# Napoliee/Expressive-FastSpeech2-Mandarin

Measured on AMD Instinct MI355X. Metric: mel-frames/sec/GPU (batch-64 synth) at 1/2/4/8 MI355X; RTF, higher is better.
Workload: dtype bf16; 1 GPU; cfg2: batch=64 x 64 phonemes per GPU, ESD-Chinese-Singing-MFA model.yaml, FastSpeech2.forward eval bf16; global_batch=64, seq_len=64, mel_frames_per_gpu_batch=24883, T_max=430, parallelism=dp1 (independent shards, no collective), hip_graph=True

## Files before the change

### expressive-fastspeech2-mandarin_amd/csrc/enc_block.hip

```cpp
#include "cond.h"
#include "fs2_common.h"

namespace {

typedef __amdgpu_buffer_rsrc_t rsrc_t;
typedef short s16x4 __attribute__((ext_vector_type(4)));

constexpr int D = 256, NQKV = 768, LMAX = 64, DK = 128, NT = 512;
constexpr int kUnit = 4096;

__device__ __forceinline__ rsrc_t rsrc(const void *p, uint32_t bytes) {
  return __builtin_amdgcn_make_buffer_rsrc(const_cast<void *>(p), (short)0, (int)bytes, 0x00020000);
}
__device__ __forceinline__ int kv_swz(int row) { return ((row & 7) << 1) | ((row >> 3) & 1); }
__device__ __forceinline__ int kv_off(int row, int chunk) { return row * 256 + ((chunk ^ kv_swz(row)) << 4); }
__device__ __forceinline__ float max_nn(float a, float b) { return __builtin_fmaxf(a, b); }
__device__ __forceinline__ float rows_sum(float v) {
  auto a = __builtin_amdgcn_permlane16_swap(__float_as_uint(v), __float_as_uint(v), false, false);
  const float s1 = __uint_as_float(a[0]) + __uint_as_float(a[1]);
  auto b = __builtin_amdgcn_permlane32_swap(__float_as_uint(s1), __float_as_uint(s1), false, false);
  return __uint_as_float(b[0]) + __uint_as_float(b[1]);
}
__device__ __forceinline__ float rows_max(float v) {
  auto a = __builtin_amdgcn_permlane16_swap(__float_as_uint(v), __float_as_uint(v), false, false);
  const float s1 = max_nn(__uint_as_float(a[0]), __uint_as_float(a[1]));
  auto b = __builtin_amdgcn_permlane32_swap(__float_as_uint(s1), __float_as_uint(s1), false, false);
  return max_nn(__uint_as_float(b[0]), __uint_as_float(b[1]));
}

__device__ __forceinline__ void bar() {
  __builtin_amdgcn_s_waitcnt(0xC07F);
  __builtin_amdgcn_sched_barrier(0);
  __builtin_amdgcn_s_barrier();
  __builtin_amdgcn_sched_barrier(0);
}

struct EncBlockArgs {
  const bf16 *x;
  const int64_t *lens;
  int B, L;
  const bf16 *wqkv;
  const float *bqkv;
  const bf16 *wfc;
  const float *bfc, *gamma, *beta;
  float eps, scale_log2;
  bf16 *out;
  const int64_t *tokens;
  const float *emb, *pe;
  int vocab, T_mel;
  int32_t *bad;
  uint8_t *src_mask;
  const int64_t *mel_lens;
  uint8_t *mel_mask;
  int *cnt;
  char *part;
  uint32_t part_bytes;
  CondArgs cond;
  int ncond, ncx;
};

constexpr int XP = D * 2 + 16;
constexpr int QP = DK * 2 + 16;
constexpr int X_OFF = 0;
constexpr int Q_OFF = X_OFF + LMAX * XP;
constexpr int K_OFF = Q_OFF + 2 * LMAX * QP;
constexpr int V_OFF = K_OFF + 2 * LMAX * 256;
constexpr int RED_OFF = V_OFF + 2 * LMAX * 256;
constexpr int VEC_OFF = RED_OFF + 2 * LMAX * 8 * 4;
constexpr int SMEM = VEC_OFF + (NQKV + 3 * D) * 4;
static_assert(2 * LMAX * QP >= LMAX * XP, "o fits the Q region");
static_assert(SMEM <= 163840, "LDS");

#ifndef ENC_TRACE
#define ENC_TRACE 0
#endif

__device__ __attribute__((noinline)) void cond_role(const CondArgs &a, int bx, int by, int tid, float *sm) {
  cond_tile(a, bx, by, tid, sm);
}

template <bool EMBED, bool COND = false>
__global__ __launch_bounds__(NT, 1) void enc_attn_block_kernel(EncBlockArgs p) {
  __shared__ __attribute__((aligned(16))) char smem[SMEM];
  uint64_t tst[10];
  int ntst = 0;
  auto stamp = [&]() {
    if (ENC_TRACE) {
      __builtin_amdgcn_sched_barrier(0);
      tst[ntst++] = __builtin_readcyclecounter();
      __builtin_amdgcn_sched_barrier(0);
    }
  };
// ... 590 lines not shown
#pragma unroll
      for (int mb = 0; mb < 4; ++mb)
        other[i][mb] = __builtin_bit_cast(f32x4, __builtin_amdgcn_raw_buffer_load_b128(pr, pofs(hh ^ 1, i, mb), 0, 16));
#pragma unroll
    for (int i = 0; i < 2; ++i)
#pragma unroll
      for (int mb = 0; mb < 4; ++mb) fa[i][mb] = hh == 0 ? fa[i][mb] + other[i][mb] : other[i][mb] + fa[i][mb];
  }
  float *red = reinterpret_cast<float *>(smem + RED_OFF);
  float part[4];
#pragma unroll
  for (int mb = 0; mb < 4; ++mb) {
    const int m = 16 * mb + li;
    float sm = 0.f;
#pragma unroll
    for (int i = 0; i < 2; ++i) {
      const int n = 16 * (2 * w + i) + 4 * g;
      const float4 bb = *reinterpret_cast<const float4 *>(vfc + n);
      const bf16x4 xv = *reinterpret_cast<const bf16x4 *>(smem + X_OFF + m * XP + n * 2);
      f32x4 v = fa[i][mb];
      v[0] = v[0] + bb.x + (float)xv[0];
      v[1] = v[1] + bb.y + (float)xv[1];
      v[2] = v[2] + bb.z + (float)xv[2];
      v[3] = v[3] + bb.w + (float)xv[3];
      fa[i][mb] = v;
      sm += (v[0] + v[1]) + (v[2] + v[3]);
    }
    part[mb] = rows_sum(sm);
  }
  auto reduce = [&](float (&pv)[4], float (&tot)[4], int pass) {
    float *rb = red + pass * LMAX * 8;
    if (g == 0) {
#pragma unroll
      for (int mb = 0; mb < 4; ++mb) rb[(16 * mb + li) * 8 + w] = pv[mb];
    }
    bar();
#pragma unroll
    for (int mb = 0; mb < 4; ++mb) {
      const float4 a = *reinterpret_cast<const float4 *>(rb + (16 * mb + li) * 8);
      const float4 c = *reinterpret_cast<const float4 *>(rb + (16 * mb + li) * 8 + 4);
      tot[mb] = ((a.x + a.y) + (a.z + a.w)) + ((c.x + c.y) + (c.z + c.w));
    }
  };
  float mean[4], var[4];
  reduce(part, mean, 0);
#pragma unroll
  for (int mb = 0; mb < 4; ++mb) {
    mean[mb] *= 1.0f / D;
    float sm = 0.f;
#pragma unroll
    for (int i = 0; i < 2; ++i) {
      f32x4 d = fa[i][mb];
#pragma unroll
      for (int j = 0; j < 4; ++j) d[j] -= mean[mb];
      fa[i][mb] = d;
      sm += (d[0] * d[0] + d[1] * d[1]) + (d[2] * d[2] + d[3] * d[3]);
    }
    part[mb] = rows_sum(sm);
  }
  reduce(part, var, 1);
#pragma unroll
  for (int mb = 0; mb < 4; ++mb) {
    const int m = 16 * mb + li;
    const float rstd = 1.0f / sqrtf(var[mb] * (1.0f / D) + p.eps);
    const float keep = m < len ? 1.0f : 0.0f;
#pragma unroll
    for (int i = 0; i < 2; ++i) {
      const int n = 16 * (2 * w + i) + 4 * g;
      const float4 gg = *reinterpret_cast<const float4 *>(vg + n);
      const float4 be = *reinterpret_cast<const float4 *>(vb + n);
      const f32x4 d = fa[i][mb];
      const bf16x4 o = {(bf16)((d[0] * rstd * gg.x + be.x) * keep), (bf16)((d[1] * rstd * gg.y + be.y) * keep),
                        (bf16)((d[2] * rstd * gg.z + be.z) * keep), (bf16)((d[3] * rstd * gg.w + be.w) * keep)};
      *reinterpret_cast<bf16x4 *>(smem + X_OFF + m * XP + n * 2) = o;
    }
  }
  __builtin_amdgcn_s_waitcnt(0xC07F);
  bar();
  uint4 *orow = reinterpret_cast<uint4 *>(p.out + (size_t)xrow0 * D);
  for (int i = tid; i < L * (D * 2 / 16); i += NT) {
    const int m = i >> 5, c = i & 31;
    orow[i] = *reinterpret_cast<const uint4 *>(smem + X_OFF + m * XP + c * 16);
  }
}

}

static int enc_block_launch(const void *x, const int64_t *tokens, const float *emb, int vocab, const float *pe,
                            int32_t *bad_ids, const int64_t *lens, int B, int L, const void *wqkv, const float *bqkv,
                            const void *wfc, const float *bfc, const float *gamma, const float *beta, float eps, int H,
                            int dk, float temperature, void *out, uint8_t *src_mask, const int64_t *mel_lens, int T_mel,
                            uint8_t *mel_mask, const fs2_cond_desc *cond, void *ws, int64_t ws_bytes,
                            fs2_stream_t stream) {
  const bool embed = tokens != nullptr;
  if ((!embed && x == nullptr) || (embed && (emb == nullptr || pe == nullptr || vocab <= 0)) || lens == nullptr ||
      wqkv == nullptr || bqkv == nullptr || wfc == nullptr || bfc == nullptr || gamma == nullptr || beta == nullptr ||
      out == nullptr || !(temperature > 0.f))
    return FS2_EINVAL;
  if (B < 0 || L < 0 || (mel_mask != nullptr && (mel_lens == nullptr || T_mel < 0))) return FS2_EINVAL;
  if (H != 2 || dk != DK || L > LMAX) return FS2_EUNSUPPORTED;
  if (x == out) return FS2_EINVAL;
  if (B == 0 || L == 0) return FS2_OK;
  if ((int64_t)B * L * D * 2 >= (1LL << 31)) return FS2_EUNSUPPORTED;
  EncBlockArgs a{};
  a.x = reinterpret_cast<const bf16 *>(x);
  a.lens = lens;
  a.B = B;
  a.L = L;
  a.wqkv = reinterpret_cast<const bf16 *>(wqkv);
  a.bqkv = bqkv;
  a.wfc = reinterpret_cast<const bf16 *>(wfc);
  a.bfc = bfc;
  a.gamma = gamma;
  a.beta = beta;
  a.eps = eps;
  a.scale_log2 = 1.4426950408889634f / temperature;
  a.out = reinterpret_cast<bf16 *>(out);
  a.tokens = tokens;
  a.emb = emb;
  a.pe = pe;
  a.vocab = vocab;
  a.bad = bad_ids;
  a.src_mask = src_mask;
  a.mel_lens = mel_lens;
  a.T_mel = T_mel;
  a.mel_mask = mel_mask;
  a.cnt = reinterpret_cast<int *>(ws);
  a.part = ws != nullptr ? static_cast<char *>(ws) + 4096 : nullptr;
  a.part_bytes = (uint32_t)(ws_bytes > 4096 ? ws_bytes - 4096 : 0);
  a.ncond = a.ncx = 0;
  if (cond != nullptr && (cond->speaker_table != nullptr || cond->emo_table != nullptr)) {
    if (!embed) return FS2_EINVAL;
    if (cond->speaker_table != nullptr && (cond->speakers == nullptr || cond->spk_out == nullptr || cond->n_speaker <= 0))
      return FS2_EINVAL;
    if (cond->emo_table != nullptr &&
        (cond->emotions == nullptr || cond->arousals == nullptr || cond->valences == nullptr || cond->aro_table == nullptr ||
         cond->val_table == nullptr || cond->lin_w == nullptr || cond->lin_b == nullptr || cond->emo_out == nullptr ||
         cond->n_emo <= 0 || cond->n_aro <= 0 || cond->n_val <= 0))
      return FS2_EINVAL;
    const int dc = cond->emo_table != nullptr ? cond->d_emo + cond->d_aro + cond->d_val : 0;
    if ((int64_t)kCondU * (dc + 256) * 4 > SMEM) return FS2_EUNSUPPORTED;
    a.cond = CondArgs{cond->speakers, cond->speaker_table, cond->n_speaker, cond->emotions, cond->emo_table, cond->n_emo,
                      cond->d_emo, cond->arousals, cond->aro_table, cond->n_aro, cond->d_aro, cond->valences,
                      cond->val_table, cond->n_val, cond->d_val, cond->lin_w, cond->lin_b, B, D, cond->spk_out,
                      cond->emo_out};
    a.ncx = D / 64;
    a.ncond = a.ncx * ((B + kCondU - 1) / kCondU);
  }
  const bool half = !ENC_TRACE && a.ncond == 0 && ws != nullptr && B <= 1024 &&
                    (int64_t)B * 2 * 65536 + 4096 <= ws_bytes;
  const unsigned nhalf = (unsigned)(((B + 7) / 8) * 16);
  if (half && embed)
    hipLaunchKernelGGL(enc_attn_half_kernel<true>, dim3(nhalf), dim3(NT), 0, as_stream(stream), a);
  else if (half)
    hipLaunchKernelGGL(enc_attn_half_kernel<false>, dim3(nhalf), dim3(NT), 0, as_stream(stream), a);
  else if (embed && a.ncond > 0)
    hipLaunchKernelGGL((enc_attn_block_kernel<true, true>), dim3((unsigned)(B + a.ncond)), dim3(NT), 0,
                       as_stream(stream), a);
  else if (embed)
    hipLaunchKernelGGL(enc_attn_block_kernel<true>, dim3((unsigned)B), dim3(NT), 0, as_stream(stream), a);
  else
    hipLaunchKernelGGL(enc_attn_block_kernel<false>, dim3((unsigned)B), dim3(NT), 0, as_stream(stream), a);
  FS2_CHECK_LAUNCH();
  return FS2_OK;
}

extern "C" int fs2_enc_attn_block(const void *x, const int64_t *lens, int B, int L, const void *wqkv, const float *bqkv,
                                  const void *wfc, const float *bfc, const float *gamma, const float *beta, float eps,
                                  int H, int dk, float temperature, void *out, void *ws, int64_t ws_bytes,
                                  fs2_stream_t stream) {
  return enc_block_launch(x, nullptr, nullptr, 0, nullptr, nullptr, lens, B, L, wqkv, bqkv, wfc, bfc, gamma, beta, eps, H,
                          dk, temperature, out, nullptr, nullptr, 0, nullptr, nullptr, ws, ws_bytes, stream);
}

extern "C" int fs2_enc_embed_attn_block(const int64_t *tokens, const float *emb, int vocab, const float *pe,
                                        int32_t *bad_ids, const int64_t *lens, int B, int L, const void *wqkv,
                                        const float *bqkv, const void *wfc, const float *bfc, const float *gamma,
                                        const float *beta, float eps, int H, int dk, float temperature, void *out,
                                        uint8_t *src_mask, const int64_t *mel_lens, int T_mel, uint8_t *mel_mask,
                                        const fs2_cond_desc *cond, void *ws, int64_t ws_bytes, fs2_stream_t stream) {
  if (tokens == nullptr) return FS2_EINVAL;
  return enc_block_launch(nullptr, tokens, emb, vocab, pe, bad_ids, lens, B, L, wqkv, bqkv, wfc, bfc, gamma, beta, eps,
                          H, dk, temperature, out, src_mask, mel_lens, T_mel, mel_mask, cond, ws, ws_bytes, stream);
}
```

### expressive-fastspeech2-mandarin_amd/csrc/ffn_wide.hip

```cpp
#include <cstdlib>
#include <type_traits>
#include <utility>

#include "conv_common.h"
#include "fs2_common.h"

#ifndef WIDE_TRACE
#define WIDE_TRACE 0
#endif

namespace {

constexpr int kWD = 256;
constexpr int kWUnit = 4096;
constexpr int kWLgkm0 = 0xC07F;

template <int N, typename Fn, int... I>
__device__ __forceinline__ void wfor_impl(Fn &&f, std::integer_sequence<int, I...>) {
  (f(std::integral_constant<int, I>{}), ...);
}
template <int N, typename Fn>
__device__ __forceinline__ void wfor(Fn &&f) {
  wfor_impl<N>(f, std::make_integer_sequence<int, N>{});
}
// ... 165 lines not shown
#pragma unroll
    for (int mb = 0; mb < MB; ++mb) acc[jb][mb] = f32x4{0.f, 0.f, 0.f, 0.f};
  auto issue = [&](auto CI, auto TI, bf16x8 (&f)[MB]) {
    constexpr int c = decltype(CI)::value, t = decltype(TI)::value, off = (c % NSLOT) * CH;
#pragma unroll
    for (int mb = 0; mb < MB; ++mb) {
      uint32_t a;
      asm volatile("v_bfe_u32 %0, %1, %2, 16" : "=v"(a) : "v"(adp[t][mb >> 1]), "n"((mb & 1) * 16));
      f[mb] = *reinterpret_cast<const bf16x8 *>(smem + a + off);
    }
  };
  auto mma = [&](const bf16x8 (&fa)[2], const bf16x8 (&fb)[MB]) {
#pragma unroll
    for (int mb = 0; mb < MB; ++mb)
#pragma unroll
      for (int jb = 0; jb < 2; ++jb)
        acc[jb][mb] = __builtin_amdgcn_mfma_f32_16x16x32_bf16(fa[jb], fb[mb], acc[jb][mb], 0, 0, 0);
  };
  bf16x8 f0[MB], f1[MB];
  issue(std::integral_constant<int, 0>{}, std::integral_constant<int, 0>{}, f0);
  wfor<NCH>([&](auto CI) {
    constexpr int c = decltype(CI)::value;
    wfor<KS>([&](auto TI) {
      constexpr int t = decltype(TI)::value;
      constexpr int kk = c * KS + t;
      if constexpr (t + 1 < KS) {
        if constexpr (kk & 1)
          issue(CI, std::integral_constant<int, t + 1>{}, f0);
        else
          issue(CI, std::integral_constant<int, t + 1>{}, f1);
      } else if constexpr (c + 1 < NCH) {
        wait_chunk(std::integral_constant<int, c + 1>{});
        if constexpr (c + 2 < NCH) dma_chunk(std::integral_constant<int, c + 2>{});
        if constexpr (kk & 1)
          issue(std::integral_constant<int, c + 1>{}, std::integral_constant<int, 0>{}, f0);
        else
          issue(std::integral_constant<int, c + 1>{}, std::integral_constant<int, 0>{}, f1);
      }
      if constexpr (kk & 1)
        mma(pa[kk % RD], f1);
      else
        mma(pa[kk % RD], f0);
      if constexpr (kk + RD < NK) load_at(std::integral_constant<int, kk + RD>{});
    });
  });
  __builtin_amdgcn_s_waitcnt(kWLgkm0);
  __builtin_amdgcn_s_barrier();
  st.at();

  constexpr int HP = 144;
  const int hrow0 = rh * 128 + r16;
#pragma unroll
  for (int jb = 0; jb < 2; ++jb) {
    const float4 bb = jb == 0 ? bb0 : bb1;
#pragma unroll
    for (int mb = 0; mb < MB; ++mb) {
      const f32x4 v = acc[jb][mb];
      bf16x4 o;
      o[0] = (bf16)fmaxf(v[0] + bb.x, 0.f);
      o[1] = (bf16)fmaxf(v[1] + bb.y, 0.f);
      o[2] = (bf16)fmaxf(v[2] + bb.z, 0.f);
      o[3] = (bf16)fmaxf(v[3] + bb.w, 0.f);
      *reinterpret_cast<bf16x4 *>(smem + (hrow0 + 16 * mb) * HP + (hh * 32 + jb * 16 + 4 * hi) * 2) = o;
    }
  }
  __builtin_amdgcn_s_waitcnt(kWLgkm0);
  __syncthreads();
  const uint32_t hrow = (uint32_t)p.F * 2u;
  char *hb = reinterpret_cast<char *>(p.h);
#pragma unroll
  for (int i = 0; i < BM * 8 / 256; ++i) {
    const int e = tid + 256 * i, r = e >> 3, c = e & 7;
    if (m0 + r < M)
      *reinterpret_cast<uint4 *>(hb + (uint32_t)(m0 + r) * hrow + (uint32_t)(slice * 128 + c * 16)) =
          *reinterpret_cast<const uint4 *>(smem + r * HP + c * 16);
  }
  if (WIDE_TRACE) {
    asm volatile("s_waitcnt vmcnt(0)" ::: "memory");
    st.at();
    st.put(p.trace, L);
  }
}

template <int F>
__global__ __launch_bounds__(256, 1) void ffn_out_kernel(WideArgs p) {
  constexpr int NK = F / 32;
  constexpr int KW = NK / 4;
  constexpr int RED = 4 * 16 * 64 * 16;
  constexpr int VEC = RED;
  constexpr int OP = kWD * 2 + 16;
  static_assert(64 * OP <= RED, "staging fits");
  __shared__ __attribute__((aligned(16))) char smem[RED + 2048 + 16];
  Stamps st;
  st.at();

  const int tid = threadIdx.x, lane = tid & 63;
  const int w = __builtin_amdgcn_readfirstlane(tid >> 6);
  const int L = (blockIdx.x & 7) * (gridDim.x >> 3) + (blockIdx.x >> 3);
  const int tile = L >> 2, q = L & 3;
  if (tile >= p.ntiles) return;
  const int M = p.rows_dev != nullptr ? min(*p.rows_dev, p.M) : p.M;
  const int m0 = tile * 64;
  if (m0 >= M) return;
  const int T = p.T;
  const int hi = lane >> 4, r16 = lane & 15;
  if (w < 2)
    __builtin_amdgcn_raw_ptr_buffer_load_lds(make_rsrc(w == 0 ? p.gamma : p.beta, 1024),
                                             (__attribute__((address_space(3))) void *)(smem + VEC + w * 1024), 16,
                                             (uint32_t)lane * 16u, 0, 0, 0);

  const rsrc_t wr = make_rsrc(p.w, p.w_bytes);
  const rsrc_t hr = make_rsrc(p.h, p.h_bytes);
  bf16x8 wa[KW][4], hb[KW][4];
  const uint32_t wb = p.w_bytes - (uint32_t)(kWD * F * 2) + (uint32_t)((q * NK + w * KW) * kWUnit) + (uint32_t)lane * 16u;
  const uint32_t hrow = (uint32_t)F * 2u;
#pragma unroll
  for (int k = 0; k < KW; ++k) {
#pragma unroll
    for (int jb = 0; jb < 4; ++jb)
      wa[k][jb] = __builtin_bit_cast(bf16x8, __builtin_amdgcn_raw_buffer_load_b128(wr, wb + k * kWUnit + jb * 1024, 0, 0));
#pragma unroll
    for (int mb = 0; mb < 4; ++mb) {
      const int m = m0 + mb * 16 + r16;
      hb[k][mb] = __builtin_bit_cast(
          bf16x8, __builtin_amdgcn_raw_buffer_load_b128(
                      hr, m < M ? (uint32_t)m * hrow + (uint32_t)((w * KW + k) * 64 + hi * 16) : kOOB, 0, 0));
    }
  }
  const int m = m0 + 16 * w + r16;
  const bool mok = m < M;
  const rsrc_t xr = make_rsrc(p.x, p.x_bytes);
  const rsrc_t zr = make_rsrc(p.z, p.z_bytes);
  float4 b2v[4];
  uint2 xv[4];
#pragma unroll
  for (int jb = 0; jb < 4; ++jb) {
    const int n = 64 * q + 16 * jb + 4 * hi;
    b2v[jb] = *reinterpret_cast<const float4 *>(p.b2 + n);
    xv[jb] = bload8(xr, mok ? (uint32_t)m * (uint32_t)p.xs * 2u + (uint32_t)n * 2u : kOOB);
  }
  __builtin_amdgcn_sched_barrier(0);
  if (WIDE_TRACE) {
    asm volatile("s_waitcnt vmcnt(0)" ::: "memory");
    st.at();
  }
  f32x4 acc[4][4];
#pragma unroll
  for (int jb = 0; jb < 4; ++jb)
#pragma unroll
    for (int mb = 0; mb < 4; ++mb) acc[jb][mb] = f32x4{0.f, 0.f, 0.f, 0.f};
#pragma unroll
  for (int k = 0; k < KW; ++k)
#pragma unroll
    for (int mb = 0; mb < 4; ++mb)
#pragma unroll
      for (int jb = 0; jb < 4; ++jb)
        acc[jb][mb] = __builtin_amdgcn_mfma_f32_16x16x32_bf16(wa[k][jb], hb[k][mb], acc[jb][mb], 0, 0, 0);
  f32x4 *red = reinterpret_cast<f32x4 *>(smem);
#pragma unroll
  for (int jb = 0; jb < 4; ++jb)
#pragma unroll
    for (int mb = 0; mb < 4; ++mb) red[(w * 16 + jb * 4 + mb) * 64 + lane] = acc[jb][mb];
  __builtin_amdgcn_s_waitcnt(kWLgkm0);
  __builtin_amdgcn_s_barrier();
  st.at();
  f32x4 zv[4];
#pragma unroll
  for (int jb = 0; jb < 4; ++jb) {
    f32x4 s = red[(0 * 16 + jb * 4 + w) * 64 + lane];
#pragma unroll
    for (int ww = 1; ww < 4; ++ww) s += red[(ww * 16 + jb * 4 + w) * 64 + lane];
    zv[jb] = s;
  }
#pragma unroll
  for (int jb = 0; jb < 4; ++jb) {
    const int n = 64 * q + 16 * jb + 4 * hi;
    const bf16x4 x4 = __builtin_bit_cast(bf16x4, xv[jb]);
    f32x4 v = zv[jb];
    v[0] = v[0] + b2v[jb].x + (float)x4[0];
    v[1] = v[1] + b2v[jb].y + (float)x4[1];
    v[2] = v[2] + b2v[jb].z + (float)x4[2];
    v[3] = v[3] + b2v[jb].w + (float)x4[3];
    __builtin_amdgcn_raw_buffer_store_b128(__builtin_bit_cast(__attribute__((ext_vector_type(4))) unsigned, v), zr,
                                           mok ? ((uint32_t)m * kWD + (uint32_t)n) * 4u : kOOB, 0, 16);
  }
  asm volatile("s_waitcnt vmcnt(0)" ::: "memory");
  __syncthreads();
  st.at();
  int *flag = reinterpret_cast<int *>(smem + RED + 2048);
  if (tid == 0) {
    const int old = __hip_atomic_fetch_add(p.cnt + tile, 1, __ATOMIC_RELAXED, __HIP_MEMORY_SCOPE_AGENT);
    const int last = old == 3;
    if (last) __hip_atomic_store(p.cnt + tile, 0, __ATOMIC_RELAXED, __HIP_MEMORY_SCOPE_AGENT);
    *flag = last;
  }
  __syncthreads();
  st.at();
  if (!*flag) {
    st.put(p.trace, L);
    return;
  }

  if (mok) {
    f32x4 v[16];
#pragma unroll
    for (int i = 0; i < 16; ++i)
      v[i] = __builtin_bit_cast(f32x4, __builtin_amdgcn_raw_buffer_load_b128(
                                           zr, ((uint32_t)m * kWD + (uint32_t)(16 * i + 4 * hi)) * 4u, 0, 16));
    bool masked = false;
    int bb = 0;
    if (p.row_pos == nullptr) {
      bb = m / T;
      masked = p.lens != nullptr && (int64_t)(m - bb * T) >= p.lens[bb];
    }
    float4 a1[16], a2[16];
#pragma unroll
    for (int i = 0; i < 16; ++i) {
      const int n = 16 * i + 4 * hi;
      a1[i] = p.av1 != nullptr ? *reinterpret_cast<const float4 *>(p.av1 + (int64_t)bb * kWD + n) : make_float4(0.f, 0.f, 0.f, 0.f);
    }
    float s = 0.f;
#pragma unroll
    for (int i = 0; i < 16; ++i) s += (v[i][0] + v[i][1]) + (v[i][2] + v[i][3]);
    s += __shfl_xor(s, 16, 64);
    s += __shfl_xor(s, 32, 64);
    const float mean = s * (1.0f / 256.0f);
    float ss = 0.f;
#pragma unroll
    for (int i = 0; i < 16; ++i) {
      v[i] -= mean;
      ss += (v[i][0] * v[i][0] + v[i][1] * v[i][1]) + (v[i][2] * v[i][2] + v[i][3] * v[i][3]);
    }
    ss += __shfl_xor(ss, 16, 64);
    ss += __shfl_xor(ss, 32, 64);
    const float rstd = 1.0f / sqrtf(ss * (1.0f / 256.0f) + p.eps);
#pragma unroll
    for (int i = 0; i < 16; ++i) {
      const int n = 16 * i + 4 * hi;
      a2[i] = p.av2 != nullptr ? *reinterpret_cast<const float4 *>(p.av2 + (int64_t)bb * kWD + n) : make_float4(0.f, 0.f, 0.f, 0.f);
    }
    const float *vg = reinterpret_cast<const float *>(smem + VEC), *vb = vg + kWD;
#pragma unroll
    for (int i = 0; i < 16; ++i) {
      const int n = 16 * i + 4 * hi;
      const float4 g = *reinterpret_cast<const float4 *>(vg + n);
      const float4 be = *reinterpret_cast<const float4 *>(vb + n);
      float y[4] = {v[i][0] * rstd * g.x + be.x, v[i][1] * rstd * g.y + be.y, v[i][2] * rstd * g.z + be.z,
                    v[i][3] * rstd * g.w + be.w};
      if (masked) y[0] = y[1] = y[2] = y[3] = 0.f;
      if (p.av1 != nullptr) {
        y[0] += a1[i].x; y[1] += a1[i].y; y[2] += a1[i].z; y[3] += a1[i].w;
      }
      if (p.av2 != nullptr) {
        y[0] += a2[i].x; y[1] += a2[i].y; y[2] += a2[i].z; y[3] += a2[i].w;
      }
      const bf16x4 o = {(bf16)y[0], (bf16)y[1], (bf16)y[2], (bf16)y[3]};
      *reinterpret_cast<bf16x4 *>(smem + (16 * w + r16) * OP + n * 2) = o;
    }
  }
  __builtin_amdgcn_s_waitcnt(kWLgkm0);
  __builtin_amdgcn_s_barrier();
#pragma unroll
  for (int i = 0; i < 8; ++i) {
    const int e = tid + 256 * i, r = e >> 5, c = e & 31;
    if (m0 + r < M)
      *reinterpret_cast<uint4 *>(p.out + (int64_t)(m0 + r) * p.os + c * 8) =
          *reinterpret_cast<const uint4 *>(smem + r * OP + c * 16);
  }
  if (WIDE_TRACE) {
    asm volatile("s_waitcnt vmcnt(0)" ::: "memory");
    st.at();
    st.put(p.trace, L);
  }
}

}

extern "C" int fs2_ffn_wide(const fs2_ffn_desc *d, void *hidden, int64_t hidden_bytes, fs2_stream_t stream) {
  if (d == nullptr || d->x == nullptr || d->w == nullptr || d->b1 == nullptr || d->b2 == nullptr ||
      d->ln_gamma == nullptr || d->ln_beta == nullptr || d->out == nullptr || hidden == nullptr)
    return FS2_EINVAL;
  if (d->B < 0 || d->T < 0 || d->x_row_stride < kWD || (d->x_row_stride & 7) || d->out_row_stride < kWD ||
      (d->out_row_stride & 7))
    return FS2_EINVAL;
  if (d->D != kWD || !(d->F == 1024 || d->F == 512) || !(d->KS == 9 || d->KS == 3) || d->pad < 0 ||
      d->pad > d->KS - 1)
    return FS2_EUNSUPPORTED;
  if (d->wqkv != nullptr || d->pre_att != nullptr) return FS2_EUNSUPPORTED;
  if ((d->rows_dev == nullptr) != (d->row_pos == nullptr)) return FS2_EINVAL;
  if (d->rows_dev != nullptr && (d->lens != nullptr || d->addvec1 != nullptr || d->addvec2 != nullptr))
    return FS2_EINVAL;
  if (d->x == d->out || hidden == d->x || hidden == d->out) return FS2_EINVAL;
  const int64_t M64 = (int64_t)d->B * d->T;
  if (M64 > 0x7fffff00LL || d->rows_max < 0) return FS2_EINVAL;
  if (M64 == 0) return FS2_OK;
  const int64_t Mg = (d->rows_dev != nullptr && d->rows_max > 0 && d->rows_max < M64) ? d->rows_max : M64;
  const int64_t xb = M64 * d->x_row_stride * 2;
  const int64_t wb = ((int64_t)d->F * d->KS * kWD + (int64_t)kWD * d->F) * 2;
  const int64_t hb = Mg * d->F * 2;
  const int ntiles64 = (int)((Mg + 63) / 64);
  const int64_t zb = Mg * kWD * 4;
  if (xb >= (1LL << 31) || hb >= (1LL << 31) || hidden_bytes < hb) return FS2_EUNSUPPORTED;
  if (d->splitk_ws == nullptr || ntiles64 > 1024 || d->splitk_ws_bytes < 4096 + zb || zb >= (1LL << 31))
    return FS2_EINVAL;
  WideArgs p{};
  p.x = reinterpret_cast<const bf16 *>(d->x);
  p.xs = d->x_row_stride;
  p.x_bytes = (uint32_t)xb;
  p.w = reinterpret_cast<const bf16 *>(d->w);
  p.w_bytes = (uint32_t)wb;
  p.b1 = d->b1;
  p.b2 = d->b2;
  p.gamma = d->ln_gamma;
  p.beta = d->ln_beta;
  p.eps = d->ln_eps;
  p.lens = d->lens;
  p.av1 = d->addvec1;
  p.av2 = d->addvec2;
  p.rows_dev = d->rows_dev;
  p.row_pos = reinterpret_cast<const int2 *>(d->row_pos);
  p.M = (int)Mg;
  p.T = d->T;
  p.pad = d->pad;
  p.F = d->F;
  p.h = static_cast<bf16 *>(hidden);
  p.h_bytes = (uint32_t)hb;
  p.cnt = static_cast<int *>(d->splitk_ws);
  p.z = reinterpret_cast<float *>(static_cast<char *>(d->splitk_ws) + 4096);
  p.z_bytes = (uint32_t)zb;
  p.out = static_cast<bf16 *>(d->out);
  p.os = d->out_row_stride;
  if (WIDE_TRACE)
    p.trace = reinterpret_cast<uint64_t *>(static_cast<char *>(d->splitk_ws) + d->splitk_ws_bytes - 65536);
  hipStream_t s = as_stream(stream);
  p.nslices = d->F / 64;
  p.ntiles = (int)((Mg + 255) / 256);
  const int n1 = (p.nslices * p.ntiles + 7) & ~7;
  constexpr int kCUs = 256;
  const size_t solo = 32 * 1024;
  if (d->KS == 9)
    hipLaunchKernelGGL((ffn_hidden_kernel<9>), dim3(n1), dim3(256), n1 <= kCUs ? solo : 0, s, p);
  else
    hipLaunchKernelGGL((ffn_hidden_kernel<3>), dim3(n1), dim3(256), n1 <= kCUs ? solo : 0, s, p);
  FS2_CHECK_LAUNCH();
  p.ntiles = ntiles64;
  if (WIDE_TRACE) p.trace += 4096;
  const int n2 = (ntiles64 * 4 + 7) & ~7;
  if (d->F == 1024)
    hipLaunchKernelGGL((ffn_out_kernel<1024>), dim3(n2), dim3(256), 0, s, p);
  else
    hipLaunchKernelGGL((ffn_out_kernel<512>), dim3(n2), dim3(256), 0, s, p);
  FS2_CHECK_LAUNCH();
  return FS2_OK;
}
```

Before: 17.87 million mel-frames/s.

## Add row-split encoder attention and row-tiled FFN output kernels for small batches

Adds an encoder attention-block kernel that splits each sequence into four 16-row query blocks, so one batch launches about four times as many workgroups. Each block recomputes the full K/V projection but only its own Q rows, then does attention, output projection and LayerNorm. Also adds an FFN output kernel that tiles by 16 or 32 rows with the K reduction split across waves through LDS, instead of a split-K global workspace, and factors the LayerNorm epilogue into a shared helper. Both target small M where the existing kernels underfill the 256 CUs, at the cost of redundant K/V projection work and extra LDS reductions. Both are chosen by default and can be turned off with environment variables.

```diff
diff --git a/expressive-fastspeech2-mandarin_amd/csrc/enc_block.hip b/expressive-fastspeech2-mandarin_amd/csrc/enc_block.hip
--- a/expressive-fastspeech2-mandarin_amd/csrc/enc_block.hip
+++ b/expressive-fastspeech2-mandarin_amd/csrc/enc_block.hip
@@ -1,3 +1,5 @@
+#include <cstdlib>
+
 #include "cond.h"
 #include "fs2_common.h"
 
@@ -8,6 +10,7 @@
 
 constexpr int D = 256, NQKV = 768, LMAX = 64, DK = 128, NT = 512;
 constexpr int kUnit = 4096;
+constexpr int kRowsMaxB = 64;
 
 __device__ __forceinline__ rsrc_t rsrc(const void *p, uint32_t bytes) {
   return __builtin_amdgcn_make_buffer_rsrc(const_cast<void *>(p), (short)0, (int)bytes, 0x00020000);
@@ -764,6 +767,322 @@
     const int m = i >> 5, c = i & 31;
     orow[i] = *reinterpret_cast<const uint4 *>(smem + X_OFF + m * XP + c * 16);
   }
+}
+
+template <bool EMBED>
+__global__ __launch_bounds__(NT, 1) void enc_attn_rows_kernel(EncBlockArgs p) {
+  __shared__ __attribute__((aligned(16))) char smem[SMEM];
+  const int tid = threadIdx.x, lane = tid & 63;
+  const int w = __builtin_amdgcn_readfirstlane(tid >> 6);
+  const int g = lane >> 4, li = lane & 15;
+  const int bid = (blockIdx.x & 7) * (gridDim.x >> 3) + (blockIdx.x >> 3);
+  const int b = bid >> 2, q = bid & 3, L = p.L;
+  if (b >= p.B || 16 * q >= L) return;
+  const int64_t len64 = p.lens[b];
+  const int len = (int)(len64 < 0 ? 0 : (len64 > L ? L : len64));
+  const uint32_t xrow0 = (uint32_t)b * (uint32_t)L;
+  const int nrow = min(16, L - 16 * q);
+  uint4 *orow = reinterpret_cast<uint4 *>(p.out + ((size_t)xrow0 + 16 * q) * D);
+
+  if constexpr (EMBED) {
+    if (q == 0) {
+      if (p.src_mask != nullptr)
+        for (int t = tid; t < L; t += NT) p.src_mask[(int64_t)b * L + t] = (int64_t)t >= len64 ? 1 : 0;
+      if (p.mel_mask != nullptr) {
+        const int64_t ml = p.mel_lens[b];
+        for (int t = tid; t < p.T_mel; t += NT) p.mel_mask[(int64_t)b * p.T_mel + t] = (int64_t)t >= ml ? 1 : 0;
+      }
+    }
+  }
+  if (16 * q >= len) {
+    if constexpr (EMBED) {
+      if (q == 0 && p.bad != nullptr && tid < L) {
+        const int64_t tok = p.tokens[xrow0 + tid];
+        if (tok < 0 || tok >= p.vocab) atomicAdd(p.bad, 1);
+      }
+    }
+    if (tid < nrow * 32) orow[tid] = make_uint4(0u, 0u, 0u, 0u);
+    return;
+  }
+
+  if constexpr (!EMBED) {
+    const rsrc_t xr = rsrc(p.x, (uint32_t)p.B * (uint32_t)L * D * 2u);
+    for (int pc = w; pc < LMAX * XP / 1024; pc += 8) {
+      const int o = pc * 1024 + lane * 16, r = o / XP, within = o - r * XP;
+      const bool ok = r < L && within < D * 2;
+      __builtin_amdgcn_raw_ptr_buffer_load_lds(xr, (__attribute__((address_space(3))) void *)(smem + X_OFF + pc * 1024),
+                                               16, ok ? (xrow0 + r) * (uint32_t)(D * 2) + (uint32_t)within : 0x80000000u,
+                                               0, 0, 0);
+    }
+  }
+  if (w < 6) {
+    const float *src = w < 3 ? p.bqkv + 256 * w : w == 3 ? p.bfc : w == 4 ? p.gamma : p.beta;
+    __builtin_amdgcn_raw_ptr_buffer_load_lds(rsrc(src, 1024), (__attribute__((address_space(3))) void *)(smem + VEC_OFF + w * 1024),
+                                             16, (uint32_t)lane * 16u, 0, 0, 0);
+  }
+  const float *vqkv = reinterpret_cast<const float *>(smem + VEC_OFF);
+  const float *vfc = vqkv + NQKV, *vg = vfc + D, *vb = vg + D;
+
+  constexpr int NKV = 4, NQ = 2, NB1 = NKV + NQ, RING = 4;
+  const rsrc_t wq = rsrc(p.wqkv, (uint32_t)NQKV * D * 2u);
+  bf16x8 ring[RING][NB1];
+  auto gblock = [&](int i) { return i < NKV ? 16 + NKV * w + i : NQ * w + (i - NKV); };
+  auto wload = [&](int ks, bf16x8 (&dst)[NB1]) {
+    __builtin_amdgcn_sched_barrier(0);
+#pragma unroll
+    for (int i = 0; i < NB1; ++i) {
+      const int nb = gblock(i);
+      auto v = __builtin_amdgcn_raw_buffer_load_b128(
+          wq, (uint32_t)lane * 16u + (uint32_t)(nb & 3) * 1024u, (uint32_t)(((nb >> 2) * (D / 32) + ks) * kUnit), 0);
+      dst[i] = __builtin_bit_cast(bf16x8, v);
+    }
+    __builtin_amdgcn_sched_barrier(0);
+  };
+#pragma unroll
+  for (int ks = 0; ks < RING; ++ks) wload(ks, ring[ks]);
+  if constexpr (EMBED) {
+    for (int i = tid; i < LMAX * (D / 8); i += NT) {
+      const int r = i >> 5, c = (i & 31) * 8;
+      bf16x8 o;
+      if (r < L) {
+        const int64_t tok = p.tokens[xrow0 + r];
+        if (tok < 0 || tok >= p.vocab) {
+#pragma unroll
+          for (int k = 0; k < 8; ++k) o[k] = (bf16)__builtin_nanf("");
+          if (p.bad != nullptr && c == 0 && q == 0) atomicAdd(p.bad, 1);
+        } else {
+          float v[8], e[8];
+          load8(p.emb + tok * D + c, v);
+          load8(p.pe + (int64_t)r * D + c, e);
+#pragma unroll
+          for (int k = 0; k < 8; ++k) o[k] = (bf16)(v[k] + e[k]);
+        }
+      } else {
+#pragma unroll
+        for (int k = 0; k < 8; ++k) o[k] = (bf16)0.f;
+      }
+      *reinterpret_cast<bf16x8 *>(smem + X_OFF + r * XP + c * 2) = o;
+    }
+  }
+  asm volatile("s_waitcnt vmcnt(%0)" ::"n"((RING - 1) * NB1) : "memory");
+  __builtin_amdgcn_s_waitcnt(0xC07F);
+  bar();
+
+  f32x4 acc[NKV][4], qacc[NQ];
+#pragma unroll
+  for (int i = 0; i < NKV; ++i)
+#pragma unroll
+    for (int mb = 0; mb < 4; ++mb) acc[i][mb] = f32x4{0.f, 0.f, 0.f, 0.f};
+#pragma unroll
+  for (int i = 0; i < NQ; ++i) qacc[i] = f32x4{0.f, 0.f, 0.f, 0.f};
+  const int mq = 16 * q + li;
+#pragma unroll
+  for (int ks = 0; ks < D / 32; ++ks) {
+    bf16x8 xf[4];
+#pragma unroll
+    for (int mb = 0; mb < 4; ++mb)
+      xf[mb] = *reinterpret_cast<const bf16x8 *>(smem + X_OFF + (16 * mb + li) * XP + ks * 64 + g * 16);
+    const bf16x8 xq = *reinterpret_cast<const bf16x8 *>(smem + X_OFF + mq * XP + ks * 64 + g * 16);
+#pragma unroll
+    for (int i = 0; i < NKV; ++i)
+#pragma unroll
+      for (int mb = 0; mb < 4; ++mb)
+        acc[i][mb] = __builtin_amdgcn_mfma_f32_16x16x32_bf16(ring[ks % RING][i], xf[mb], acc[i][mb], 0, 0, 0);
+#pragma unroll
+    for (int i = 0; i < NQ; ++i)
+      qacc[i] = __builtin_amdgcn_mfma_f32_16x16x32_bf16(ring[ks % RING][NKV + i], xq, qacc[i], 0, 0, 0);
+    if (ks + RING < D / 32) wload(ks + RING, ring[ks % RING]);
+  }
+#pragma unroll
+  for (int i = 0; i < NKV; ++i) {
+    const int n = 16 * gblock(i) + 4 * g;
+    const float4 bb = *reinterpret_cast<const float4 *>(vqkv + n);
+    const int part = n >> 8, hh = (n >> 7) & 1, dim = n & 127;
+#pragma unroll
+    for (int mb = 0; mb < 4; ++mb) {
+      const int m = 16 * mb + li;
+      const f32x4 v = acc[i][mb];
+      const bf16x4 o = {(bf16)(v[0] + bb.x), (bf16)(v[1] + bb.y), (bf16)(v[2] + bb.z), (bf16)(v[3] + bb.w)};
+      *reinterpret_cast<bf16x4 *>(smem + (part == 1 ? K_OFF : V_OFF) + hh * LMAX * 256 + kv_off(m, dim >> 3) + (dim & 7) * 2) = o;
+    }
+  }
+#pragma unroll
+  for (int i = 0; i < NQ; ++i) {
+    const int n = 16 * gblock(NKV + i) + 4 * g;
+    const float4 bb = *reinterpret_cast<const float4 *>(vqkv + n);
+    const int hh = (n >> 7) & 1, dim = n & 127;
+    const f32x4 v = qacc[i];
+    const bf16x4 o = {(bf16)(v[0] + bb.x), (bf16)(v[1] + bb.y), (bf16)(v[2] + bb.z), (bf16)(v[3] + bb.w)};
+    *reinterpret_cast<bf16x4 *>(smem + Q_OFF + (hh * LMAX + mq) * QP + dim * 2) = o;
+  }
+  __builtin_amdgcn_s_waitcnt(0xC07F);
+  bar();
+
+  const rsrc_t wf = rsrc(p.wfc, (uint32_t)D * D * 2u);
+  bf16x8 fw[D / 32][2];
+#pragma unroll
+  for (int ks = 0; ks < D / 32; ++ks)
+#pragma unroll
+    for (int i = 0; i < 2; ++i) {
+      const int nb = 2 * w + i;
+      fw[ks][i] = __builtin_bit_cast(bf16x8, __builtin_amdgcn_raw_buffer_load_b128(
+                                                 wf, (uint32_t)lane * 16u + (uint32_t)(nb & 3) * 1024u,
+                                                 (uint32_t)(((nb >> 2) * (D / 32) + ks) * kUnit), 0));
+    }
+  f32x4 oacc[DK / 16];
+  float l_run = 0.f;
+  if (w < 2) {
+    const int h = w;
+    bf16x8 qf[4];
+#pragma unroll
+    for (int s = 0; s < 4; ++s)
+      qf[s] = *reinterpret_cast<const bf16x8 *>(smem + Q_OFF + (h * LMAX + mq) * QP + (32 * s + 8 * g) * 2);
+#pragma unroll
+    for (int i = 0; i < DK / 16; ++i) oacc[i] = f32x4{0.f, 0.f, 0.f, 0.f};
+    const char *Kb = smem + K_OFF + h * LMAX * 256;
+    const char *Vb = smem + V_OFF + h * LMAX * 256;
+    constexpr int NBK = LMAX / 16;
+    f32x4 sacc[NBK];
+#pragma unroll
+    for (int ni = 0; ni < NBK; ++ni) {
+      sacc[ni] = f32x4{0.f, 0.f, 0.f, 0.f};
+#pragma unroll
+      for (int s = 0; s < 4; ++s) {
+        const bf16x8 kf = *reinterpret_cast<const bf16x8 *>(Kb + kv_off(ni * 16 + li, 4 * s + g));
+        sacc[ni] = __builtin_amdgcn_mfma_f32_16x16x32_bf16(kf, qf[s], sacc[ni], 0, 0, 0);
+      }
+    }
+    const int lim = len - 4 * g;
+#pragma unroll
+    for (int ni = 0; ni < NBK; ++ni)
+#pragma unroll
+      for (int j = 0; j < 4; ++j)
+        if (ni * 16 + j >= lim) sacc[ni][j] = -INFINITY;
+    float mx = -INFINITY;
+#pragma unroll
+    for (int ni = 0; ni < NBK; ++ni) {
+      mx = max_nn(max_nn(mx, sacc[ni][0]), sacc[ni][1]);
+      mx = max_nn(max_nn(mx, sacc[ni][2]), sacc[ni][3]);
+    }
+    const float m_new = rows_max(mx);
+    const float mc = -m_new * p.scale_log2;
+    float sx = 0.f, sy = 0.f;
+    bf16x8 pf[NBK / 2];
+#pragma unroll
+    for (int ni = 0; ni < NBK; ++ni)
+#pragma unroll
+      for (int jp = 0; jp < 2; ++jp) {
+        const float px = __builtin_amdgcn_exp2f(__builtin_fmaf(sacc[ni][2 * jp], p.scale_log2, mc));
+        const float py = __builtin_amdgcn_exp2f(__builtin_fmaf(sacc[ni][2 * jp + 1], p.scale_log2, mc));
+        sx += px;
+        sy += py;
+        pf[ni >> 1][(ni & 1) * 4 + 2 * jp] = (bf16)px;
+        pf[ni >> 1][(ni & 1) * 4 + 2 * jp + 1] = (bf16)py;
+      }
+    l_run = rows_sum(sx + sy);
+    const int tq = li >> 2, tp = li & 3;
+#pragma unroll
+    for (int s2 = 0; s2 < NBK / 2; ++s2) {
+#pragma unroll
+      for (int h4 = 0; h4 < DK / 64; ++h4) {
+        bf16x8 vf[4];
+#pragma unroll
+        for (int i = 0; i < 4; ++i) {
+          const int nd = 4 * h4 + i;
+          const char *vp = Vb + kv_off(4 * g + tq, nd * 2 + (tp >> 1)) + (tp & 1) * 8 + s2 * 32 * 256;
+          auto lo = __builtin_amdgcn_ds_read_tr16_b64_v4i16((__attribute__((address_space(3))) s16x4 *)vp);
+          auto hi = __builtin_amdgcn_ds_read_tr16_b64_v4i16((__attribute__((address_space(3))) s16x4 *)(vp + 16 * 256));
+          __builtin_memcpy(&vf[i], &lo, 8);
+          __builtin_memcpy(reinterpret_cast<char *>(&vf[i]) + 8, &hi, 8);
+        }
+#pragma unroll
+        for (int i = 0; i < 4; ++i)
+          oacc[4 * h4 + i] = __builtin_amdgcn_mfma_f32_16x16x32_bf16(vf[i], pf[s2], oacc[4 * h4 + i], 0, 0, 0);
+      }
+    }
+  }
+  __builtin_amdgcn_s_waitcnt(0xC07F);
+  bar();
+  if (w < 2) {
+    const float inv = l_run > 0.f ? 1.0f / l_run : 0.f;
+#pragma unroll
+    for (int nd = 0; nd < DK / 16; ++nd) {
+      const bf16x4 o = {(bf16)(oacc[nd][0] * inv), (bf16)(oacc[nd][1] * inv), (bf16)(oacc[nd][2] * inv),
+                        (bf16)(oacc[nd][3] * inv)};
+      *reinterpret_cast<bf16x4 *>(smem + Q_OFF + mq * XP + (w * DK + nd * 16 + 4 * g) * 2) = o;
+    }
+  }
+  __builtin_amdgcn_s_waitcnt(0xC07F);
+  bar();
+
+  f32x4 fa[2];
+#pragma unroll
+  for (int i = 0; i < 2; ++i) fa[i] = f32x4{0.f, 0.f, 0.f, 0.f};
+#pragma unroll
+  for (int ks = 0; ks < D / 32; ++ks) {
+    const bf16x8 of = *reinterpret_cast<const bf16x8 *>(smem + Q_OFF + mq * XP + ks * 64 + g * 16);
+#pragma unroll
+    for (int i = 0; i < 2; ++i) fa[i] = __builtin_amdgcn_mfma_f32_16x16x32_bf16(fw[ks][i], of, fa[i], 0, 0, 0);
+  }
+  float *red = reinterpret_cast<float *>(smem + RED_OFF);
+  float part;
+  {
+    float s = 0.f;
+#pragma unroll
+    for (int i = 0; i < 2; ++i) {
+      const int n = 16 * (2 * w + i) + 4 * g;
+      const float4 bb = *reinterpret_cast<const float4 *>(vfc + n);
+      const bf16x4 xv = *reinterpret_cast<const bf16x4 *>(smem + X_OFF + mq * XP + n * 2);
+      f32x4 v = fa[i];
+      v[0] = v[0] + bb.x + (float)xv[0];
+      v[1] = v[1] + bb.y + (float)xv[1];
+      v[2] = v[2] + bb.z + (float)xv[2];
+      v[3] = v[3] + bb.w + (float)xv[3];
+      fa[i] = v;
+      s += (v[0] + v[1]) + (v[2] + v[3]);
+    }
+    part = rows_sum(s);
+  }
+  auto reduce = [&](float pv, int pass) {
+    float *rb = red + pass * LMAX * 8;
+    if (g == 0) rb[mq * 8 + w] = pv;
+    bar();
+    const float4 a = *reinterpret_cast<const float4 *>(rb + mq * 8);
+    const float4 c = *reinterpret_cast<const float4 *>(rb + mq * 8 + 4);
+    return ((a.x + a.y) + (a.z + a.w)) + ((c.x + c.y) + (c.z + c.w));
+  };
+  float mean = reduce(part, 0);
+  {
+    mean *= 1.0f / D;
+    float s = 0.f;
+#pragma unroll
+    for (int i = 0; i < 2; ++i) {
+      f32x4 d = fa[i];
+#pragma unroll
+      for (int j = 0; j < 4; ++j) d[j] -= mean;
+      fa[i] = d;
+      s += (d[0] * d[0] + d[1] * d[1]) + (d[2] * d[2] + d[3] * d[3]);
+    }
+    part = rows_sum(s);
+  }
+  const float var = reduce(part, 1);
+  {
+    const float rstd = 1.0f / sqrtf(var * (1.0f / D) + p.eps);
+    const float keep = mq < len ? 1.0f : 0.0f;
+#pragma unroll
+    for (int i = 0; i < 2; ++i) {
+      const int n = 16 * (2 * w + i) + 4 * g;
+      const float4 gg = *reinterpret_cast<const float4 *>(vg + n);
+      const float4 be = *reinterpret_cast<const float4 *>(vb + n);
+      const f32x4 d = fa[i];
+      const bf16x4 o = {(bf16)((d[0] * rstd * gg.x + be.x) * keep), (bf16)((d[1] * rstd * gg.y + be.y) * keep),
+                        (bf16)((d[2] * rstd * gg.z + be.z) * keep), (bf16)((d[3] * rstd * gg.w + be.w) * keep)};
+      *reinterpret_cast<bf16x4 *>(smem + X_OFF + mq * XP + n * 2) = o;
+    }
+  }
+  __builtin_amdgcn_s_waitcnt(0xC07F);
+  bar();
+  if (tid < nrow * 32) orow[tid] = *reinterpret_cast<const uint4 *>(smem + X_OFF + (16 * q + (tid >> 5)) * XP + (tid & 31) * 16);
 }
 
 }
@@ -832,7 +1151,14 @@
   const bool half = !ENC_TRACE && a.ncond == 0 && ws != nullptr && B <= 1024 &&
                     (int64_t)B * 2 * 65536 + 4096 <= ws_bytes;
   const unsigned nhalf = (unsigned)(((B + 7) / 8) * 16);
-  if (half && embed)
+  const char *erows = getenv("FS2_ENC_ROWS");
+  const bool rows = !ENC_TRACE && a.ncond == 0 && ws == nullptr && B <= kRowsMaxB && !(erows != nullptr && erows[0] == '0');
+  const unsigned nrows = (unsigned)((4 * B + 31) & ~31);
+  if (rows && embed)
+    hipLaunchKernelGGL(enc_attn_rows_kernel<true>, dim3(nrows), dim3(NT), 0, as_stream(stream), a);
+  else if (rows)
+    hipLaunchKernelGGL(enc_attn_rows_kernel<false>, dim3(nrows), dim3(NT), 0, as_stream(stream), a);
+  else if (half && embed)
     hipLaunchKernelGGL(enc_attn_half_kernel<true>, dim3(nhalf), dim3(NT), 0, as_stream(stream), a);
   else if (half)
     hipLaunchKernelGGL(enc_attn_half_kernel<false>, dim3(nhalf), dim3(NT), 0, as_stream(stream), a);
diff --git a/expressive-fastspeech2-mandarin_amd/csrc/ffn_wide.hip b/expressive-fastspeech2-mandarin_amd/csrc/ffn_wide.hip
--- a/expressive-fastspeech2-mandarin_amd/csrc/ffn_wide.hip
+++ b/expressive-fastspeech2-mandarin_amd/csrc/ffn_wide.hip
@@ -271,6 +271,200 @@
   }
 }
 
+__device__ __forceinline__ void ln_row(const WideArgs &p, f32x4 (&v)[16], int m, int hi, const char *vec, char *dst) {
+  bool masked = false;
+  int bb = 0;
+  if (p.row_pos == nullptr) {
+    bb = m / p.T;
+    masked = p.lens != nullptr && (int64_t)(m - bb * p.T) >= p.lens[bb];
+  }
+  float4 a1[16], a2[16];
+#pragma unroll
+  for (int i = 0; i < 16; ++i) {
+    const int n = 16 * i + 4 * hi;
+    a1[i] = p.av1 != nullptr ? *reinterpret_cast<const float4 *>(p.av1 + (int64_t)bb * kWD + n) : make_float4(0.f, 0.f, 0.f, 0.f);
+  }
+  float s = 0.f;
+#pragma unroll
+  for (int i = 0; i < 16; ++i) s += (v[i][0] + v[i][1]) + (v[i][2] + v[i][3]);
+  s += __shfl_xor(s, 16, 64);
+  s += __shfl_xor(s, 32, 64);
+  const float mean = s * (1.0f / 256.0f);
+  float ss = 0.f;
+#pragma unroll
+  for (int i = 0; i < 16; ++i) {
+    v[i] -= mean;
+    ss += (v[i][0] * v[i][0] + v[i][1] * v[i][1]) + (v[i][2] * v[i][2] + v[i][3] * v[i][3]);
+  }
+  ss += __shfl_xor(ss, 16, 64);
+  ss += __shfl_xor(ss, 32, 64);
+  const float rstd = 1.0f / sqrtf(ss * (1.0f / 256.0f) + p.eps);
+#pragma unroll
+  for (int i = 0; i < 16; ++i) {
+    const int n = 16 * i + 4 * hi;
+    a2[i] = p.av2 != nullptr ? *reinterpret_cast<const float4 *>(p.av2 + (int64_t)bb * kWD + n) : make_float4(0.f, 0.f, 0.f, 0.f);
+  }
+  const float *vg = reinterpret_cast<const float *>(vec), *vb = vg + kWD;
+#pragma unroll
+  for (int i = 0; i < 16; ++i) {
+    const int n = 16 * i + 4 * hi;
+    const float4 g = *reinterpret_cast<const float4 *>(vg + n);
+    const float4 be = *reinterpret_cast<const float4 *>(vb + n);
+    float y[4] = {v[i][0] * rstd * g.x + be.x, v[i][1] * rstd * g.y + be.y, v[i][2] * rstd * g.z + be.z,
+                  v[i][3] * rstd * g.w + be.w};
+    if (masked) y[0] = y[1] = y[2] = y[3] = 0.f;
+    if (p.av1 != nullptr) {
+      y[0] += a1[i].x; y[1] += a1[i].y; y[2] += a1[i].z; y[3] += a1[i].w;
+    }
+    if (p.av2 != nullptr) {
+      y[0] += a2[i].x; y[1] += a2[i].y; y[2] += a2[i].z; y[3] += a2[i].w;
+    }
+    const bf16x4 o = {(bf16)y[0], (bf16)y[1], (bf16)y[2], (bf16)y[3]};
+    *reinterpret_cast<bf16x4 *>(dst + n * 2) = o;
+  }
+}
+
+template <int F, int RB>
+__global__ __launch_bounds__(256, 1) void ffn_out_rows_kernel(WideArgs p) {
+  constexpr int NK = F / 32;
+  constexpr int KW = NK / 4;
+  constexpr int BM = 16 * RB;
+  constexpr int RD = 3;
+  static_assert(KW >= RD && (RD - 1) * (16 + RB) <= 63, "ring");
+  constexpr int RED = 4 * 16 * RB * 64 * 16;
+  constexpr int ZP = kWD * 4 + 64;
+  constexpr int ZB = BM * ZP;
+  constexpr int OP = kWD * 2 + 16;
+  constexpr int VEC = RED;
+  static_assert(ZB + BM * OP <= RED, "pre-norm rows + staging fit over the partials");
+  static_assert(RED + 2048 <= 163840, "LDS");
+  __shared__ __attribute__((aligned(16))) char smem[RED + 2048];
+  Stamps st;
+  st.at();
+
+  const int tid = threadIdx.x, lane = tid & 63;
+  const int w = __builtin_amdgcn_readfirstlane(tid >> 6);
+  const int L = (blockIdx.x & 7) * (gridDim.x >> 3) + (blockIdx.x >> 3);
+  if (L >= p.ntiles) return;
+  const int M = p.rows_dev != nullptr ? min(*p.rows_dev, p.M) : p.M;
+  const int m0 = L * BM;
+  if (m0 >= M) return;
+  const int hi = lane >> 4, r16 = lane & 15;
+  if (w < 2)
+    __builtin_amdgcn_raw_ptr_buffer_load_lds(make_rsrc(w == 0 ? p.gamma : p.beta, 1024),
+                                             (__attribute__((address_space(3))) void *)(smem + VEC + w * 1024), 16,
+                                             (uint32_t)lane * 16u, 0, 0, 0);
+  const rsrc_t xr = make_rsrc(p.x, p.x_bytes);
+  float4 b2v[4];
+  uint2 xv[RB][4];
+#pragma unroll
+  for (int jb = 0; jb < 4; ++jb) {
+    const int n = 64 * w + 16 * jb + 4 * hi;
+    b2v[jb] = *reinterpret_cast<const float4 *>(p.b2 + n);
+#pragma unroll
+    for (int mb = 0; mb < RB; ++mb) {
+      const int m = m0 + 16 * mb + r16;
+      xv[mb][jb] = bload8(xr, m < M ? (uint32_t)m * (uint32_t)p.xs * 2u + (uint32_t)n * 2u : kOOB);
+    }
+  }
+
+  const rsrc_t wr = make_rsrc(p.w, p.w_bytes);
+  const rsrc_t hr = make_rsrc(p.h, p.h_bytes);
+  const uint32_t wb = p.w_bytes - (uint32_t)(kWD * F * 2) + (uint32_t)(w * KW * kWUnit) + (uint32_t)lane * 16u;
+  const uint32_t hrow = (uint32_t)F * 2u;
+  uint32_t hoff[RB];
+#pragma unroll
+  for (int mb = 0; mb < RB; ++mb) {
+    const int m = m0 + 16 * mb + r16;
+    hoff[mb] = m < M ? (uint32_t)m * hrow + (uint32_t)(w * KW * 64 + hi * 16) : kOOB;
+  }
+  bf16x8 wa[RD][16], hb[RD][RB];
+  auto load_at = [&](auto KI) {
+    constexpr int k = decltype(KI)::value;
+    __builtin_amdgcn_sched_barrier(0);
+#pragma unroll
+    for (int J = 0; J < 16; ++J)
+      wa[k % RD][J] = __builtin_bit_cast(
+          bf16x8, __builtin_amdgcn_raw_buffer_load_b128(wr, wb + (uint32_t)(((J >> 2) * NK + k) * kWUnit + (J & 3) * 1024), 0, 0));
+#pragma unroll
+    for (int mb = 0; mb < RB; ++mb)
+      hb[k % RD][mb] = __builtin_bit_cast(bf16x8, __builtin_amdgcn_raw_buffer_load_b128(hr, hoff[mb] + (uint32_t)(k * 64), 0, 0));
+    __builtin_amdgcn_sched_barrier(0);
+  };
+  wfor<RD>([&](auto I) { load_at(I); });
+  if (WIDE_TRACE) st.at();
+
+  f32x4 acc[16][RB];
+#pragma unroll
+  for (int J = 0; J < 16; ++J)
+#pragma unroll
+    for (int mb = 0; mb < RB; ++mb) acc[J][mb] = f32x4{0.f, 0.f, 0.f, 0.f};
+  wfor<KW>([&](auto KI) {
+    constexpr int k = decltype(KI)::value;
+#pragma unroll
+    for (int mb = 0; mb < RB; ++mb)
+#pragma unroll
+      for (int J = 0; J < 16; ++J)
+        acc[J][mb] = __builtin_amdgcn_mfma_f32_16x16x32_bf16(wa[k % RD][J], hb[k % RD][mb], acc[J][mb], 0, 0, 0);
+    if constexpr (k + RD < KW) load_at(std::integral_constant<int, k + RD>{});
+  });
+  f32x4 *red = reinterpret_cast<f32x4 *>(smem);
+#pragma unroll
+  for (int J = 0; J < 16; ++J)
+#pragma unroll
+    for (int mb = 0; mb < RB; ++mb) red[((w * 16 + J) * RB + mb) * 64 + lane] = acc[J][mb];
+  asm volatile("s_waitcnt vmcnt(0)" ::: "memory");
+  __builtin_amdgcn_s_waitcnt(kWLgkm0);
+  __builtin_amdgcn_s_barrier();
+  st.at();
+  f32x4 zv[RB][4];
+#pragma unroll
+  for (int mb = 0; mb < RB; ++mb)
+#pragma unroll
+    for (int jb = 0; jb < 4; ++jb) {
+      const int J = 4 * w + jb;
+      f32x4 s = red[((0 * 16 + J) * RB + mb) * 64 + lane];
+#pragma unroll
+      for (int ww = 1; ww < 4; ++ww) s += red[((ww * 16 + J) * RB + mb) * 64 + lane];
+      const bf16x4 x4 = __builtin_bit_cast(bf16x4, xv[mb][jb]);
+      s[0] = s[0] + b2v[jb].x + (float)x4[0];
+      s[1] = s[1] + b2v[jb].y + (float)x4[1];
+      s[2] = s[2] + b2v[jb].z + (float)x4[2];
+      s[3] = s[3] + b2v[jb].w + (float)x4[3];
+      zv[mb][jb] = s;
+    }
+  __builtin_amdgcn_s_waitcnt(kWLgkm0);
+  __builtin_amdgcn_s_barrier();
+#pragma unroll
+  for (int mb = 0; mb < RB; ++mb)
+#pragma unroll
+    for (int jb = 0; jb < 4; ++jb)
+      *reinterpret_cast<f32x4 *>(smem + (16 * mb + r16) * ZP + (64 * w + 16 * jb + 4 * hi) * 4) = zv[mb][jb];
+  __builtin_amdgcn_s_waitcnt(kWLgkm0);
+  __builtin_amdgcn_s_barrier();
+  st.at();
+  if (w < RB && m0 + 16 * w + r16 < M) {
+    f32x4 v[16];
+#pragma unroll
+    for (int i = 0; i < 16; ++i) v[i] = *reinterpret_cast<const f32x4 *>(smem + (16 * w + r16) * ZP + (16 * i + 4 * hi) * 4);
+    ln_row(p, v, m0 + 16 * w + r16, hi, smem + VEC, smem + ZB + (16 * w + r16) * OP);
+  }
+  __builtin_amdgcn_s_waitcnt(kWLgkm0);
+  __builtin_amdgcn_s_barrier();
+#pragma unroll
+  for (int i = 0; i < BM * 32 / 256; ++i) {
+    const int e = tid + 256 * i, r = e >> 5, c = e & 31;
+    if (m0 + r < M)
+      *reinterpret_cast<uint4 *>(p.out + (int64_t)(m0 + r) * p.os + c * 8) =
+          *reinterpret_cast<const uint4 *>(smem + ZB + r * OP + c * 16);
+  }
+  if (WIDE_TRACE) {
+    asm volatile("s_waitcnt vmcnt(0)" ::: "memory");
+    st.at();
+    st.put(p.trace, L);
+  }
+}
+
 template <int F>
 __global__ __launch_bounds__(256, 1) void ffn_out_kernel(WideArgs p) {
   constexpr int NK = F / 32;
@@ -291,7 +485,6 @@
   const int M = p.rows_dev != nullptr ? min(*p.rows_dev, p.M) : p.M;
   const int m0 = tile * 64;
   if (m0 >= M) return;
-  const int T = p.T;
   const int hi = lane >> 4, r16 = lane & 15;
   if (w < 2)
     __builtin_amdgcn_raw_ptr_buffer_load_lds(make_rsrc(w == 0 ? p.gamma : p.beta, 1024),
@@ -396,56 +589,7 @@
     for (int i = 0; i < 16; ++i)
       v[i] = __builtin_bit_cast(f32x4, __builtin_amdgcn_raw_buffer_load_b128(
                                            zr, ((uint32_t)m * kWD + (uint32_t)(16 * i + 4 * hi)) * 4u, 0, 16));
-    bool masked = false;
-    int bb = 0;
-    if (p.row_pos == nullptr) {
-      bb = m / T;
-      masked = p.lens != nullptr && (int64_t)(m - bb * T) >= p.lens[bb];
-    }
-    float4 a1[16], a2[16];
-#pragma unroll
-    for (int i = 0; i < 16; ++i) {
-      const int n = 16 * i + 4 * hi;
-      a1[i] = p.av1 != nullptr ? *reinterpret_cast<const float4 *>(p.av1 + (int64_t)bb * kWD + n) : make_float4(0.f, 0.f, 0.f, 0.f);
-    }
-    float s = 0.f;
-#pragma unroll
-    for (int i = 0; i < 16; ++i) s += (v[i][0] + v[i][1]) + (v[i][2] + v[i][3]);
-    s += __shfl_xor(s, 16, 64);
-    s += __shfl_xor(s, 32, 64);
-    const float mean = s * (1.0f / 256.0f);
-    float ss = 0.f;
-#pragma unroll
-    for (int i = 0; i < 16; ++i) {
-      v[i] -= mean;
-      ss += (v[i][0] * v[i][0] + v[i][1] * v[i][1]) + (v[i][2] * v[i][2] + v[i][3] * v[i][3]);
-    }
-    ss += __shfl_xor(ss, 16, 64);
-    ss += __shfl_xor(ss, 32, 64);
-    const float rstd = 1.0f / sqrtf(ss * (1.0f / 256.0f) + p.eps);
-#pragma unroll
-    for (int i = 0; i < 16; ++i) {
-      const int n = 16 * i + 4 * hi;
-      a2[i] = p.av2 != nullptr ? *reinterpret_cast<const float4 *>(p.av2 + (int64_t)bb * kWD + n) : make_float4(0.f, 0.f, 0.f, 0.f);
-    }
-    const float *vg = reinterpret_cast<const float *>(smem + VEC), *vb = vg + kWD;
-#pragma unroll
-    for (int i = 0; i < 16; ++i) {
-      const int n = 16 * i + 4 * hi;
-      const float4 g = *reinterpret_cast<const float4 *>(vg + n);
-      const float4 be = *reinterpret_cast<const float4 *>(vb + n);
-      float y[4] = {v[i][0] * rstd * g.x + be.x, v[i][1] * rstd * g.y + be.y, v[i][2] * rstd * g.z + be.z,
-                    v[i][3] * rstd * g.w + be.w};
-      if (masked) y[0] = y[1] = y[2] = y[3] = 0.f;
-      if (p.av1 != nullptr) {
-        y[0] += a1[i].x; y[1] += a1[i].y; y[2] += a1[i].z; y[3] += a1[i].w;
-      }
-      if (p.av2 != nullptr) {
-        y[0] += a2[i].x; y[1] += a2[i].y; y[2] += a2[i].z; y[3] += a2[i].w;
-      }
-      const bf16x4 o = {(bf16)y[0], (bf16)y[1], (bf16)y[2], (bf16)y[3]};
-      *reinterpret_cast<bf16x4 *>(smem + (16 * w + r16) * OP + n * 2) = o;
-    }
+    ln_row(p, v, m, hi, smem + VEC, smem + (16 * w + r16) * OP);
   }
   __builtin_amdgcn_s_waitcnt(kWLgkm0);
   __builtin_amdgcn_s_barrier();
@@ -526,14 +670,39 @@
   p.ntiles = (int)((Mg + 255) / 256);
   const int n1 = (p.nslices * p.ntiles + 7) & ~7;
   constexpr int kCUs = 256;
+  constexpr int kRowsRounds = 2;
   const size_t solo = 32 * 1024;
   if (d->KS == 9)
     hipLaunchKernelGGL((ffn_hidden_kernel<9>), dim3(n1), dim3(256), n1 <= kCUs ? solo : 0, s, p);
   else
     hipLaunchKernelGGL((ffn_hidden_kernel<3>), dim3(n1), dim3(256), n1 <= kCUs ? solo : 0, s, p);
   FS2_CHECK_LAUNCH();
+  if (WIDE_TRACE) p.trace += 4096;
+  {
+    const char *e = getenv("FS2_WIDE_OUT"), *f = getenv("FS2_WIDE_OUT_RB");
+    int rb = 0;
+    if (e == nullptr || e[0] != '0') {
+      if (f != nullptr && (f[0] == '1' || f[0] == '2'))
+        rb = f[0] - '0';
+      else
+        rb = Mg <= 16 * kCUs ? 1 : Mg <= 32 * kRowsRounds * kCUs ? 2 : 0;
+    }
+    if (rb != 0) {
+      p.ntiles = (int)((Mg + 16 * rb - 1) / (16 * rb));
+      const int nr = (p.ntiles + 7) & ~7;
+      if (d->F == 1024 && rb == 1)
+        hipLaunchKernelGGL((ffn_out_rows_kernel<1024, 1>), dim3(nr), dim3(256), 0, s, p);
+      else if (d->F == 1024)
+        hipLaunchKernelGGL((ffn_out_rows_kernel<1024, 2>), dim3(nr), dim3(256), 0, s, p);
+      else if (rb == 1)
+        hipLaunchKernelGGL((ffn_out_rows_kernel<512, 1>), dim3(nr), dim3(256), 0, s, p);
+      else
+        hipLaunchKernelGGL((ffn_out_rows_kernel<512, 2>), dim3(nr), dim3(256), 0, s, p);
+      FS2_CHECK_LAUNCH();
+      return FS2_OK;
+    }
+  }
   p.ntiles = ntiles64;
-  if (WIDE_TRACE) p.trace += 4096;
   const int n2 = (ntiles64 * 4 + 7) & ~7;
   if (d->F == 1024)
     hipLaunchKernelGGL((ffn_out_kernel<1024>), dim3(n2), dim3(256), 0, s, p);
```

Result: faster. 18.36 million mel-frames/s, median of 6 (+2.8%).
